# ziyaad30/ForwardTacotron

Hardware: AMD Instinct MI355X
Metric: mel_frames_per_sec_train_step (higher is better)
Workload: dtype f32

## Files before the change

### forwardtacotron_amd/csrc/ft_rnn_persist.hip

```cpp
#include <stdio.h>
#include <stdlib.h>
#include <string.h>

#include <mutex>
#include <vector>

#include "ft_rnn.h"

namespace {

constexpr int NSH = 16;
constexpr int CSTRIDE = 32;
constexpr unsigned MAX_SPINS_DEFAULT = 1u << 18;
constexpr int MB = 16;
constexpr int NFLAG = 256;
constexpr int NXCC = 64;

typedef unsigned int u32x4 __attribute__((ext_vector_type(4)));
typedef __bf16 bf16x8 __attribute__((ext_vector_type(8)));
typedef unsigned short u16x8 __attribute__((ext_vector_type(8)));

typedef __bf16 bf16x2v __attribute__((ext_vector_type(2)));
__device__ __forceinline__ unsigned rn_pack(float a, float b) {
  const bf16x2v p = {(__bf16)a, (__bf16)b};
  return __builtin_bit_cast(unsigned, p);
}
__device__ __forceinline__ void split_pair(float a, float b, unsigned& hi, unsigned& mid, unsigned& lo) {
  hi = rn_pack(a, b);
  const float a1 = a - __uint_as_float(hi << 16), b1 = b - __uint_as_float(hi & 0xFFFF0000u);
// ... 147 lines not shown
    same &= __hip_atomic_load(ids + i, __ATOMIC_RELAXED, __HIP_MEMORY_SCOPE_AGENT) == mine;
  return __all(same);
}

__device__ __forceinline__ bool decode(const Geom& g, int& d, int& bgp, int& chunk, int& grp) {
  const int lin = blockIdx.x, per = gridDim.x >> 3;
  const int w = g.xcd_aware ? (((lin & 7) + 8 - g.xcd_off) & 7) * per + (lin >> 3) : lin;
  if (w >= g.total) return false;
  grp = w / g.nchunks;
  chunk = w - grp * g.nchunks;
  d = grp / g.nbg;
  bgp = grp - d * g.nbg;
  return true;
}

template <int G, int NW, bool B3, int UB, int BC>
__global__ __launch_bounds__(NW * 64, NW == 4 ? 2 : 1) void ft_rnn_fwd_persist_kernel(RnnFwdArgs a, Geom geo, float* xb, unsigned* cnt,
                                                                     unsigned* fault, unsigned xb_bytes) {
  constexpr int NT = (G * UB + 15) / 16, BCH = BC, CW = UB / 4;
  constexpr bool GRAN = B3 && BC <= 2;
  static_assert(UB % 4 == 0 && CW <= NW, "cell waves");
  __shared__ float red2[2 * NW * NT * 16 * RLD];
  __shared__ int s_ok;
  int d, bgp, chunk, grp;
  if (!decode(geo, d, bgp, chunk, grp)) return;
  const int u0 = chunk * UB, b0 = bgp * MB;
  const int tid = threadIdx.x, wave = tid >> 6, lane = tid & 63;
  const int q = lane >> 4, l15 = lane & 15;
  const int H = a.H, T = a.T, nq = H / 4;
  const long ldo = (long)a.ND * H;
  const long ldx = (long)a.ND * G * H;
  const long grp_floats = (long)nq * MB * 4;
  const long par_floats = (long)2 * geo.nbg * grp_floats;
  const long base_floats = (long)grp * grp_floats;
  unsigned* mycnt = cnt + (long)grp * NSH * CSTRIDE;
  const int nprod = (geo.sig_per_wave ? CW : 1) * geo.nchunks;
  const __amdgpu_buffer_rsrc_t rs = __builtin_amdgcn_make_buffer_rsrc(xb, 0, (int)xb_bytes, 0x00020000);
  unsigned* myflags = cnt + (long)2 * geo.nbg * NSH * CSTRIDE + (long)grp * NFLAG;
  unsigned* myxcc = cnt + (long)2 * geo.nbg * (NSH * CSTRIDE + NFLAG) + (long)grp * NXCC;
  const unsigned my_xcc = xcc_id() + 1u;
  __shared__ int s_local, s_fail;
  bool local = false;
  if (tid == 0) {
// ... 26 lines not shown
        const bool in = valid && kb0 + c < kb1;
        const float* p = brow + (in ? 32 * (kb0 + c) + 8 * q : 0);
        const float4 z = make_float4(0, 0, 0, 0);
        split8(in ? *reinterpret_cast<const float4*>(p) : z, in ? *reinterpret_cast<const float4*>(p + 4) : z,
               bw[nt][c][0], bw[nt][c][1], bw[nt][c][2]);
      }
    }
  }

  const int pq0 = B3 ? 8 * kb0 : 4 * g0, pnq = B3 ? 8 * max(kb1 - kb0, 0) : 4 * max(g1 - g0, 0);
  const unsigned* pollf = lane < pnq ? myflags + pq0 + lane : nullptr;

  const int jq = tid >> 6, ci = (tid >> 2) & 15, jj = tid & 3;
  const int cu = 4 * jq + jj;
  const int cb = b0 + ci, cun = u0 + cu;
  const bool sthr = tid < 64 * CW;
  const bool cthr = sthr && cb < a.B;
  const int L = cthr ? clamp_len(a.lens, cb, T) : 0;
  float bg[G];
#pragma unroll
  for (int g = 0; g < G; ++g) bg[g] = sthr ? a.bhh[d][g * H + cun] : 0.f;
  float hprev = 0.f, cprev = 0.f;
  float xg[G];
#pragma unroll
  for (int g = 0; g < G; ++g) xg[g] = 0.f;
  const bool gated = a.gate != nullptr;
  int gate_off = 0;
  unsigned gate_have = 1u;
  if (gated && d == 1) {
    int lm = T;
    for (int i = 0; i < MB; ++i)
// ... 48 lines not shown
      for (int e = 0; e < 4; ++e) acc[nt][e] = 0.f;
    float4 av[B3 ? 1 : GCH];
    float4 aw[B3 ? BCH : 1][2];
    float xn[G];
#pragma unroll
    for (int g = 0; g < G; ++g) xn[g] = 0.f;
    auto request_xn = [&]() {
      if (cthr && s + 1 < L) xload(d == 0 ? s + 1 : L - 2 - s, xn);
    };
    const bool gl = local;
    const bool gm = GRAN && s > 0 && gl && geo.gran;
    const unsigned want_hi = ((unsigned)s & 0xFFFFu) << 16;
    const unsigned gbase = (unsigned)(((long)2 * par_floats * 4) + ((long)((s - 1) & 1) * par_floats + base_floats) * 8);
    auto goffs = [&](int c, unsigned& oa, unsigned& ob) {
      const long quad = 8 * (kb0 + c) + 2 * q;
      oa = gbase + (unsigned)((quad * MB + l15) * 4 * 8);
      ob = gbase + (unsigned)(((quad + 1) * MB + l15) * 4 * 8);
    };
    Gran gr[2];
    if (s > 0 && !gm) {
      if (gl) {
        if (!poll_flag(pollf, (unsigned)s, geo.max_spins) && lane == 0) s_fail = 1;
      } else {
        if (wave == 0) {
          const bool ok = wait_arrivals(mycnt, (unsigned)s, nprod, lane, geo.max_spins);
          if (s == 1 && ok && geo.local_ok) {
            const bool same = same_xcd(myxcc, geo.nchunks, my_xcc, lane);
            if (lane == 0) s_local = same;
          }
          if (lane == 0) s_ok = ok;
        }
        __syncthreads();
// ... 2 lines not shown
          return;
        }
        if (s == 1) {
          local = s_local != 0;
          if (threadIdx.x == 0 && chunk == 0) atomicAdd(fault + (local ? 8 : 9), 1u);
        }
      }
    }
    if (s > 0) {
      const long rbase = (long)((s - 1) & 1) * par_floats + base_floats;
      if constexpr (!B3) {
#pragma unroll
        for (int c = 0; c < GCH; ++c)
          if (g0 + c < g1) {
            const long quad = 4 * (g0 + c) + q;
            av[c] = ld_sc1_b128(rs, (unsigned)((rbase + (quad * MB + l15) * 4) * 4));
          }
        request_xn();
#pragma unroll
        for (int c = 0; c < GCH; ++c)
          if (g0 + c < g1) {
#pragma unroll
            for (int nt = 0; nt < NT; ++nt) mfma4(av[c], bv[nt][c], acc[nt]);
          }
      } else {
        if (gm) {
          if constexpr (GRAN) {
            if (kb0 < kb1) {
              unsigned oa, ob;
              goffs(0, oa, ob);
              gran_load(gr[0], rs, oa, ob);
            }
          }
        } else {
#pragma unroll
          for (int c = 0; c < BCH; ++c)
            if (kb0 + c < kb1) {
              const long quad = 8 * (kb0 + c) + 2 * q;
              aw[c][0] = ld_sc1_b128(rs, (unsigned)((rbase + (quad * MB + l15) * 4) * 4));
              aw[c][1] = ld_sc1_b128(rs, (unsigned)((rbase + ((quad + 1) * MB + l15) * 4) * 4));
            }
          request_xn();
        }
        bool ok = true;
#pragma unroll
        for (int c = 0; c < BCH; ++c)
          if (kb0 + c < kb1) {
            bf16x8 a3[3];
            if (gm) {
              if constexpr (GRAN) {
                unsigned oa, ob;
                if (c + 1 < BCH && kb0 + c + 1 < kb1) {
                  goffs(c + 1, oa, ob);
                  gran_load(gr[(c + 1) & 1], rs, oa, ob);
                }
// ... 57 lines not shown
      } else if (local) {
        __hip_atomic_store(xb + xe, hnew, __ATOMIC_RELAXED, __HIP_MEMORY_SCOPE_WAVEFRONT);
      } else {
        __hip_atomic_store(xb + xe, hnew, __ATOMIC_RELAXED, __HIP_MEMORY_SCOPE_AGENT);
      }
    }
    PROF(4);
    if (local && GRAN && geo.gran) {
      if (sthr) {
        const long xe = (long)(s & 1) * par_floats + base_floats + (((long)CW * chunk + jq) * MB + ci) * 4 + jj;
        unsigned long long* gp = reinterpret_cast<unsigned long long*>(xb + 2 * par_floats) + xe;
        __hip_atomic_store(gp, gran_make(cact ? hnew : 0.f, (unsigned)(s + 1) & 0xFFFFu), __ATOMIC_RELAXED,
                           __HIP_MEMORY_SCOPE_WAVEFRONT);
      }
    } else if (geo.sig_per_wave) {
      if (sthr) {
        asm volatile("s_waitcnt vmcnt(0)" ::: "memory");
        if (lane == 0) {
          if (local)
            __hip_atomic_store(myflags + CW * chunk + jq, (unsigned)(s + 1), __ATOMIC_RELAXED, __HIP_MEMORY_SCOPE_WAVEFRONT);
          else
            __hip_atomic_fetch_add(mycnt + ((CW * chunk + jq) % NSH) * CSTRIDE, 1u, __ATOMIC_RELAXED,
                                   __HIP_MEMORY_SCOPE_AGENT);
        }
      }
    } else {
      asm volatile("s_waitcnt vmcnt(0)" ::: "memory");
      __syncthreads();
      if (tid == 0)
        __hip_atomic_fetch_add(mycnt + (chunk % NSH) * CSTRIDE, 1u, __ATOMIC_RELAXED, __HIP_MEMORY_SCOPE_AGENT);
    }
// ... 13 lines not shown
    }
    PROF(6);
#pragma unroll
    for (int g = 0; g < G; ++g) xg[g] = xn[g];
    PROF(7);
  }
  PROF_DUMP(grp == 0 && chunk == 3 && wave == 0, 0);
  PROF_DUMP(grp == 0 && chunk == 3 && wave == NW - 1, 1);
}

template <int G, int NW, int GW, bool B3>
__global__ __launch_bounds__(NW * 64) void ft_rnn_bwd_persist_kernel(RnnBwdArgs a, Geom geo, float* xb, unsigned* cnt,
                                                                     unsigned* fault, unsigned xb_bytes) {
  __shared__ float red2[2 * NW * 16 * RLD];
  __shared__ int s_ok;
  int d, bgp, chunk, grp;
  if (!decode(geo, d, bgp, chunk, grp)) return;
  const int u0 = chunk * 16, b0 = bgp * MB;
  const int tid = threadIdx.x, wave = tid >> 6, lane = tid & 63;
  const int q = lane >> 4, l15 = lane & 15;
  const int H = a.H, T = a.T, K = G * H, nq = K / 4;
  const long ldg = (long)a.ND * K;
  const long ldo = (long)a.ND * H;
  const long grp_floats = (long)nq * MB * 4;
  const long par_floats = (long)2 * geo.nbg * grp_floats;
  const long base_floats = (long)grp * grp_floats;
  unsigned* mycnt = cnt + (long)grp * NSH * CSTRIDE;
  const int nprod = (geo.sig_per_wave ? 4 : 1) * geo.nchunks;
  const __amdgpu_buffer_rsrc_t rs = __builtin_amdgcn_make_buffer_rsrc(xb, 0, (int)xb_bytes, 0x00020000);
  unsigned* myflags = cnt + (long)2 * geo.nbg * NSH * CSTRIDE + (long)grp * NFLAG;
// ... 267 lines not shown
      if (G == 3) {
        float* dhh = a.dhp + ((long)s * a.B + cb) * ldg + (long)d * K + cun;
        dhh[0] = 0.f; dhh[H] = 0.f; dhh[2 * H] = 0.f;
      }
    }
    PROF(6);
#pragma unroll
    for (int g = 0; g < 4; ++g) gv[g] = ngv[g];
    dov = ndo; cc = ncc; prev = nprev;
    PROF(7);
  }
  PROF_DUMP(grp == 0 && chunk == 3 && wave == 0, 0);
  PROF_DUMP(grp == 0 && chunk == 3 && wave == 5, 1);
}

template <int G, int NW, int NT>
__global__ __launch_bounds__(NW * 64) void ft_rnn_bwd_rs_kernel(RnnBwdArgs a, Geom geo, float* xb, unsigned* cnt,
                                                                unsigned* fault, unsigned xb_bytes) {
  constexpr int ALD = 68;
  constexpr int GWV = 4;
  constexpr int TPW = NW * NT / GWV;
  constexpr bool PF = NW >= 8;
  constexpr int NIN = 7;
  __shared__ __attribute__((aligned(16))) float adg2[2 * 16 * ALD];
  __shared__ __attribute__((aligned(16))) float rsum[GWV * 256];
  __shared__ float inb[PF ? 2 * NIN * 256 : 1];
  __shared__ int s_ok;
  int d, bgp, chunk, grp;
  if (!decode(geo, d, bgp, chunk, grp)) return;
  const int u0 = chunk * 16, b0 = bgp * MB;
  const int tid = threadIdx.x, wave = tid >> 6, lane = tid & 63;
  const int q = lane >> 4, l15 = lane & 15;
  const int H = a.H, T = a.T, K = G * H, P = geo.nchunks;
  const long ldg = (long)a.ND * K;
  const long ldo = (long)a.ND * H;
  const long grp_floats = (long)P * P * 256;
  const long par_floats = (long)2 * geo.nbg * grp_floats;
  const long base_floats = (long)grp * grp_floats;
  unsigned* mycnt = cnt + (long)grp * NSH * CSTRIDE;
  const int nprod = NW * P;
  const __amdgpu_buffer_rsrc_t rs = __builtin_amdgcn_make_buffer_rsrc(xb, 0, (int)xb_bytes, 0x00020000);
  unsigned* myflags = cnt + (long)2 * geo.nbg * NSH * CSTRIDE + (long)grp * NFLAG;
  unsigned* myxcc = cnt + (long)2 * geo.nbg * (NSH * CSTRIDE + NFLAG) + (long)grp * NXCC;
  const unsigned my_xcc = xcc_id() + 1u;
  __shared__ int s_local, s_fail;
  bool local = false;
  if (threadIdx.x == 0) {
    s_local = 0;
    s_fail = 0;
    __hip_atomic_store(myxcc + chunk, my_xcc, __ATOMIC_RELAXED, __HIP_MEMORY_SCOPE_AGENT);
  }

  bf16x8 bw[NT][2][3];
#pragma unroll
  for (int nt = 0; nt < NT; ++nt) {
    const int n = (wave * NT + nt) * 16 + l15;
#pragma unroll
    for (int blk = 0; blk < 2; ++blk) {
      const int g = 2 * blk + (q >> 1), j0 = 8 * (q & 1);
      const bool in = g < G && n < H;
      const float* p = a.whhT[d] + (in ? (long)n * K + (long)g * H + u0 + j0 : 0);
      const float4 z = make_float4(0, 0, 0, 0);
      split8(in ? *reinterpret_cast<const float4*>(p) : z, in ? *reinterpret_cast<const float4*>(p + 4) : z,
             bw[nt][blk][0], bw[nt][blk][1], bw[nt][blk][2]);
    }
  }
  for (int i = tid; i < 2 * 16 * ALD; i += NW * 64) adg2[i] = 0.f;

  const unsigned* pollf =
      (wave < GWV && lane < TPW && wave * TPW + lane < P) ? myflags + NW * (wave * TPW + lane) + chunk / NT : nullptr;

  const int cj = tid >> 4, ci = tid & 15;
  const int cb = b0 + ci, cun = u0 + cj;
  const bool sthr = tid < 256;
  const bool cthr = sthr && cb < a.B;
  const int L = cthr ? clamp_len(a.lens, cb, T) : 0;
  float carry = 0.f;
  const bool fwave = PF && wave == 4;
  const int fr = lane >> 2, fq = lane & 3;
  const int fb = b0 + fr;
  const int FL = (fwave && fb < a.B) ? clamp_len(a.lens, fb, T) : 0;

  float gv[4] = {0.f, 0.f, 0.f, 0.f}, dov = 0.f, cc = 0.f, prev = 0.f;
  auto request = [&](int sn, float (&rgv)[4], float& rdo, float& rcc, float& rprev) {
#pragma unroll
    for (int g = 0; g < 4; ++g) rgv[g] = 0.f;
    rdo = 0.f; rcc = 0.f; rprev = 0.f;
    if (cthr && sn < L) {
      const int ct = d == 0 ? L - 1 - sn : sn;
      const int tprev = d == 0 ? ct - 1 : ct + 1;
      const bool has_prev = tprev >= 0 && tprev < L;
      const long o = ((long)ct * a.B + cb) * ldo + (long)d * H + cun;
      const long op = ((long)tprev * a.B + cb) * ldo + (long)d * H + cun;
      const float* gs = a.gates + (((long)ct * a.B + cb) * a.ND + d) * 4 * H + cun;
#pragma unroll
      for (int g = 0; g < 4; ++g) rgv[g] = gs[(long)g * H];
      rdo = a.dout[o];
      if (G == 3) {
        rprev = has_prev ? a.out[op] : 0.f;
      } else {
        rcc = a.cst[o];
        rprev = has_prev ? a.cst[op] : 0.f;
      }
    }
  };
  float4 fv[NIN];
#pragma unroll
  for (int i = 0; i < NIN; ++i) fv[i] = make_float4(0.f, 0.f, 0.f, 0.f);
  auto fetch = [&](int sn) {
#pragma unroll
    for (int i = 0; i < NIN; ++i) fv[i] = make_float4(0.f, 0.f, 0.f, 0.f);
    if (fwave && sn < FL) {
      const int ct = d == 0 ? FL - 1 - sn : sn;
      const int tprev = d == 0 ? ct - 1 : ct + 1;
      const bool has_prev = tprev >= 0 && tprev < FL;
      const long o = ((long)ct * a.B + fb) * ldo + (long)d * H + u0 + 4 * fq;
      const long op = ((long)tprev * a.B + fb) * ldo + (long)d * H + u0 + 4 * fq;
      const float* gs = a.gates + (((long)ct * a.B + fb) * a.ND + d) * 4 * H + u0 + 4 * fq;
#pragma unroll
      for (int g = 0; g < 4; ++g) fv[g] = *reinterpret_cast<const float4*>(gs + (long)g * H);
      fv[4] = *reinterpret_cast<const float4*>(a.dout + o);
      if (G == 3) {
        if (has_prev) fv[6] = *reinterpret_cast<const float4*>(a.out + op);
      } else {
        fv[5] = *reinterpret_cast<const float4*>(a.cst + o);
        if (has_prev) fv[6] = *reinterpret_cast<const float4*>(a.cst + op);
      }
    }
  };
  auto publish = [&](int sn) {
    if (fwave) {
      float* ib = inb + (sn & 1) * (NIN * 256) + (4 * fq) * 16 + fr;
#pragma unroll
      for (int i = 0; i < NIN; ++i) {
        ib[i * 256] = fv[i].x; ib[i * 256 + 16] = fv[i].y; ib[i * 256 + 32] = fv[i].z; ib[i * 256 + 48] = fv[i].w;
      }
    }
  };
  if constexpr (PF) {
    fetch(0);
    publish(0);
  } else {
    request(0, gv, dov, cc, prev);
  }
  __syncthreads();
  PROF_DECL;

  for (int s = 0; s < T; ++s) {
    PROF(0);
    const bool cact = cthr && s < L;
    const int ct = d == 0 ? L - 1 - s : s;
    float* adg = adg2 + (s & 1) * (16 * ALD);
    float rec = 0.f;
    if (s > 0) {
      if (local) {
        if (!poll_flag(pollf, (unsigned)s, geo.max_spins) && lane == 0) s_fail = 1;
      } else {
        if (wave == 0) {
          const bool ok = wait_arrivals(mycnt, (unsigned)s, nprod, lane, geo.max_spins);
          if (s == 1 && ok && geo.local_ok) {
            const bool same = same_xcd(myxcc, P, my_xcc, lane);
            if (lane == 0) s_local = same;
          }
          if (lane == 0) s_ok = ok;
        }
        __syncthreads();
        if (!s_ok) {
          if (tid == 0) atomicExch(fault, 1u);
          return;
        }
        if (s == 1) {
          local = s_local != 0;
          if (threadIdx.x == 0 && chunk == 0) atomicAdd(fault + (local ? 8 : 9), 1u);
        }
      }
      PROF(1);
      if (wave < GWV) {
        const long rbase = (long)((s - 1) & 1) * par_floats + base_floats + (long)chunk * P * 256 + 4 * lane;
        float4 v[TPW];
#pragma unroll
        for (int i = 0; i < TPW; ++i) {
          const int pp = wave * TPW + i;
          v[i] = pp < P ? ld_sc1_b128(rs, (unsigned)((rbase + (long)pp * 256) * 4)) : make_float4(0.f, 0.f, 0.f, 0.f);
        }
        float4 acc4 = v[0];
#pragma unroll
        for (int i = 1; i < TPW; ++i) {
          acc4.x += v[i].x; acc4.y += v[i].y; acc4.z += v[i].z; acc4.w += v[i].w;
        }
        *reinterpret_cast<float4*>(rsum + wave * 256 + 4 * lane) = acc4;
      }
      __syncthreads();
      if (sthr) {
#pragma unroll
        for (int w = 0; w < GWV; ++w) rec += rsum[w * 256 + tid];
      }
    }
    if constexpr (PF) {
      fetch(s + 1);
      if (sthr) {
        const float* ib = inb + (s & 1) * (NIN * 256) + tid;
#pragma unroll
        for (int g = 0; g < 4; ++g) gv[g] = ib[g * 256];
        dov = ib[4 * 256]; cc = ib[5 * 256]; prev = ib[6 * 256];
      }
    }
    float ngv[4] = {0.f, 0.f, 0.f, 0.f}, ndo = 0.f, ncc = 0.f, nprev = 0.f;
    if constexpr (!PF) request(s + 1, ngv, ndo, ncc, nprev);
#ifdef FT_RNN_PROF
    asm volatile("" : "+v"(rec));
#endif
    PROF(2);

    float dgx[4] = {0.f, 0.f, 0.f, 0.f}, dgh2 = 0.f;
    if (cact) {
      if (G == 3) {
        const float dh = dov + rec + carry;
        const float r = gv[0], z = gv[1], n = gv[2], hn = gv[3];
        const float dz = dh * (prev - n) * z * (1.f - z);
// ... 19 lines not shown
#pragma unroll
      for (int g = 0; g < G; ++g) adg[ci * ALD + g * 16 + cj] = (G == 3 && g == 2) ? dgh2 : dgx[g];
    }
    PROF(3);
    __syncthreads();
    PROF(4);
    if (s_fail) {
      if (tid == 0) atomicExch(fault, 1u);
      return;
    }

    if (s + 1 < T) {
      bf16x8 a3[2][3];
#pragma unroll
      for (int blk = 0; blk < 2; ++blk) {
        const float* ap = adg + l15 * ALD + 32 * blk + 8 * q;
        split8(*reinterpret_cast<const float4*>(ap), *reinterpret_cast<const float4*>(ap + 4), a3[blk][0], a3[blk][1],
               a3[blk][2]);
      }
      PROF(5);
      const long wbase = (long)(s & 1) * par_floats + base_floats + (long)chunk * 256 + l15 * 16 + 4 * q;
#pragma unroll
      for (int nt = 0; nt < NT; ++nt) {
        f32x4 acc = {0.f, 0.f, 0.f, 0.f};
        mfma6(a3[0], bw[nt][0], acc);
        mfma6(a3[1], bw[nt][1], acc);
        const int cons = wave * NT + nt;
        if (cons < P) {
          u32x4 v = {__float_as_uint(acc[0]), __float_as_uint(acc[1]), __float_as_uint(acc[2]), __float_as_uint(acc[3])};
          const unsigned off = (unsigned)((wbase + (long)cons * P * 256) * 4);
          if (local) __builtin_amdgcn_raw_buffer_store_b128(v, rs, off, 0, 0);
          else __builtin_amdgcn_raw_buffer_store_b128(v, rs, off, 0, 16);
        }
      }
      PROF(6);
      asm volatile("s_waitcnt vmcnt(0)" ::: "memory");
      PROF(7);
      if (lane == 0) {
        if (local)
          __hip_atomic_store(myflags + NW * chunk + wave, (unsigned)(s + 1), __ATOMIC_RELAXED, __HIP_MEMORY_SCOPE_WAVEFRONT);
        else
          __hip_atomic_fetch_add(mycnt + ((NW * chunk + wave) % NSH) * CSTRIDE, 1u, __ATOMIC_RELAXED,
                                 __HIP_MEMORY_SCOPE_AGENT);
      }
    }
// ... 46 lines not shown
  if (!cus) {
    int dev = 0;
    hipDeviceProp_t p;
    if (hipGetDevice(&dev) == hipSuccess && hipGetDeviceProperties(&p, dev) == hipSuccess) cus = p.multiProcessorCount;
    if (cus <= 0) cus = 1;
  }
  return cus;
}

struct PersistWs {
  float* xb;
  unsigned* cnt;
  size_t sync_bytes, xb_bytes, total_bytes;
};
size_t sync_region_bytes(int ngrp) { return (size_t)ngrp * (NSH * CSTRIDE + NFLAG + NXCC) * sizeof(unsigned); }
PersistWs carve_ws(void* ws, int ngrp, int K) {
  PersistWs p;
  p.sync_bytes = sync_region_bytes(ngrp);
  p.cnt = (unsigned*)ws;
  p.xb_bytes = (size_t)3 * 2 * ngrp * (K / 4) * MB * 4 * sizeof(float);
  p.xb = (float*)((char*)ws + p.sync_bytes);
  p.total_bytes = p.sync_bytes + p.xb_bytes;
  return p;
}

PersistWs carve_ws_rs(void* ws, int ngrp, int nchunks) {
  PersistWs p;
  p.sync_bytes = sync_region_bytes(ngrp);
  p.cnt = (unsigned*)ws;
  p.xb_bytes = (size_t)2 * ngrp * nchunks * nchunks * 256 * sizeof(float);
  p.xb = (float*)((char*)ws + p.sync_bytes);
  p.total_bytes = p.sync_bytes + p.xb_bytes;
  return p;
}

constexpr int MAX_DEV = 16;
unsigned g_max_spins = MAX_SPINS_DEFAULT;
long g_n_persistent = 0, g_n_refused = 0, g_n_waited = 0;

int current_device() {
  int dev = 0;
  if (hipGetDevice(&dev) != hipSuccess || dev < 0 || dev >= MAX_DEV) dev = 0;
  return dev;
}

struct Flight {
  hipEvent_t ev;
  hipStream_t stream;
// ... 108 lines not shown
              geo.total, geo.nchunks, cand[i].aligned ? "aligned" : "spread", cand[i].per, d, ok ? "admitted" : "refused");
    if (!ok) continue;
    grid = cand[i].grid;
    geo.xcd_off = cand[i].xcd_off;
    geo.local_ok = cand[i].aligned && env_int("FT_RNN_LOCAL", 1);
    geo.gran = env_int("FT_RNN_GRANULES", 1);
    geo.fast = env_int("FT_RNN_FAST_CELL", 1);
    return d;
  }
  ++g_n_refused;
  return -1.0;
}

double* g_fill_probe = nullptr;

template <int G, int NW, bool B3, int UB, int BC>
int launch_fwd_persist(const RnnFwdArgs& a, Geom geo, const PersistWs& p, hipStream_t stream) {
  if (g_fill_probe) {
    const int ngroups = geo.total / geo.nchunks;
    *g_fill_probe = xcd_demand(ft_rnn_fwd_persist_kernel<G, NW, B3, UB, BC>, NW * 64, geo.nchunks * ft_cdiv(ngroups, 8));
    return FT_OK;
  }
  int grid = 0;
  const double cus = plan_launch(ft_rnn_fwd_persist_kernel<G, NW, B3, UB, BC>, NW * 64, geo, grid, stream);
  if (cus < 0.0) return -1;
  if (BC > 2 && !env_int("FT_RNN_GRAN4", 1)) geo.gran = 0;
  (void)hipMemsetAsync(p.cnt, 0, p.total_bytes, stream);
  hipLaunchKernelGGL((ft_rnn_fwd_persist_kernel<G, NW, B3, UB, BC>), dim3(grid), dim3(NW * 64), 0, stream, a, geo, p.xb,
                     p.cnt, ft_rnn_fault_word(), (unsigned)p.xb_bytes);
  admitted_launch_done(cus, stream);
  return ft_check_launch("rnn_fwd_persistent");
}

template <int G>
int fwd_persistent(RnnFwdArgs a, void* ws, size_t ws_bytes, hipStream_t stream) {
  if (!persistent_enabled() || !ws || a.T < 2) return -1;
  const int H = a.H, B = a.B;
  if (!a.vec || H % 16 != 0) return -1;
  const int ngroups = H / 16;
  int NW = ngroups > 16 ? 8 : 4;
  const bool wide = NW == 8 && G == 4 && H / 8 > 32 && H % 32 == 0 && ft_cdiv(H / 32, 8) <= 2 && env_int("FT_RNN_B3", 1) &&
                    env_int("FT_RNN_FWD_UB16", 1);
  if (!wide && NW == 8 && G == 4 && H % 32 == 0 && ft_cdiv(H / 32, 4) <= 4 && env_int("FT_RNN_FWD_NW4", 1)) NW = 4;
  if (ft_cdiv(ngroups, NW) > GCH) return -1;
  const int bpw = H % 32 == 0 ? ft_cdiv(H / 32, NW) : 99;
  const bool b3 = bpw <= 4 && env_int("FT_RNN_B3", 1);
  const bool gru_wide = G == 3 && H == 256 && b3 && NW == 4 && env_int("FT_RNN_GRU_WIDE", 1);
  Geom geo;
  geo.nchunks = H / ((wide || gru_wide) ? 16 : 8);
  geo.nbg = ft_cdiv(B, MB);
  geo.total = a.ND * geo.nbg * geo.nchunks;
  geo.xcd_aware = env_int("FT_RNN_XCDMAP", 1);
  geo.sig_per_wave = env_int("FT_RNN_SIG", 1);
  geo.max_spins = g_max_spins;
  PersistWs p = carve_ws(ws, 2 * geo.nbg, H);
  if (ws_bytes < p.total_bytes || p.xb_bytes >= (1ull << 31)) return -1;
  geo.xcd_off = 0;
  geo.local_ok = 0;
  geo.gran = 0;
  geo.fast = 0;
  a.s = 0;
  if (wide) return launch_fwd_persist<G, 8, true, 16, 2>(a, geo, p, stream);
  if constexpr (G == 3) {
    if (gru_wide) return launch_fwd_persist<G, 8, true, 16, 1>(a, geo, p, stream);
  }
  if (b3) {
    if (NW == 8) return bpw <= 1 ? launch_fwd_persist<G, 8, true, 8, 1>(a, geo, p, stream)
                                 : launch_fwd_persist<G, 8, true, 8, 2>(a, geo, p, stream);
    if (bpw <= 1) return launch_fwd_persist<G, 4, true, 8, 1>(a, geo, p, stream);
    if (bpw <= 2) return launch_fwd_persist<G, 4, true, 8, 2>(a, geo, p, stream);
    return launch_fwd_persist<G, 4, true, 8, 4>(a, geo, p, stream);
  }
  return NW == 8 ? launch_fwd_persist<G, 8, false, 8, 1>(a, geo, p, stream)
                 : launch_fwd_persist<G, 4, false, 8, 1>(a, geo, p, stream);
}

// ... 2 lines not shown
  if (g_fill_probe) {
    *g_fill_probe = xcd_demand(ft_rnn_bwd_persist_kernel<G, NW, GW, B3>, NW * 64,
                               geo.nchunks * ft_cdiv(geo.total / geo.nchunks, 8));
    return FT_OK;
  }
  int grid = 0;
  const double cus = plan_launch(ft_rnn_bwd_persist_kernel<G, NW, GW, B3>, NW * 64, geo, grid, stream);
  if (cus < 0.0) return -1;
  (void)hipMemsetAsync(p.cnt, 0, p.total_bytes, stream);
  hipLaunchKernelGGL((ft_rnn_bwd_persist_kernel<G, NW, GW, B3>), dim3(grid), dim3(NW * 64), 0, stream, a, geo, p.xb, p.cnt,
                     ft_rnn_fault_word(), (unsigned)p.xb_bytes);
  admitted_launch_done(cus, stream);
  return ft_check_launch("rnn_bwd_persistent");
}

template <int G, int NW, int NT>
int launch_bwd_rs(const RnnBwdArgs& a, Geom geo, const PersistWs& p, hipStream_t stream) {
  if (g_fill_probe) {
    *g_fill_probe = xcd_demand(ft_rnn_bwd_rs_kernel<G, NW, NT>, NW * 64, geo.nchunks * ft_cdiv(geo.total / geo.nchunks, 8));
    return FT_OK;
  }
  int grid = 0;
  const double cus = plan_launch(ft_rnn_bwd_rs_kernel<G, NW, NT>, NW * 64, geo, grid, stream);
  if (cus < 0.0) return -1;
  (void)hipMemsetAsync(p.cnt, 0, p.sync_bytes, stream);
  hipLaunchKernelGGL((ft_rnn_bwd_rs_kernel<G, NW, NT>), dim3(grid), dim3(NW * 64), 0, stream, a, geo, p.xb, p.cnt,
                     ft_rnn_fault_word(), (unsigned)p.xb_bytes);
  admitted_launch_done(cus, stream);
  return ft_check_launch("rnn_bwd_persistent_rs");
}

template <int G>
int bwd_persistent_rs(RnnBwdArgs a, const Geom& geo, void* ws, size_t ws_bytes, hipStream_t stream) {
  const int tiles = a.H / 16;
  if (!env_int("FT_RNN_BWD_RS", 1) || !env_int("FT_RNN_B3", 1) || !geo.sig_per_wave) return -1;
  PersistWs p = carve_ws_rs(ws, 2 * geo.nbg, geo.nchunks);
  if (ws_bytes < p.total_bytes || p.xb_bytes >= (1ull << 31)) return -1;
  const bool force = env_int("FT_RNN_BWD_RS", 1) == 2;
  if (!force && G * a.H < 1024) return -1;
  switch (tiles) {
    case 4: return launch_bwd_rs<G, 4, 1>(a, geo, p, stream);
    case 8: return launch_bwd_rs<G, 8, 1>(a, geo, p, stream);
    case 16: return launch_bwd_rs<G, 8, 2>(a, geo, p, stream);
    case 32: return launch_bwd_rs<G, 8, 4>(a, geo, p, stream);
    default: return -1;
  }
}

template <int G>
int bwd_persistent(RnnBwdArgs a, void* ws, size_t ws_bytes, hipStream_t stream) {
  if (!persistent_enabled() || !ws || a.T < 2) return -1;
  const int H = a.H, B = a.B, K = G * H;
  if (!a.vec || H % 16 != 0) return -1;
  const int ngroups = K / 16;
  const int NW = ngroups > 128 ? 16 : (ngroups > 16 ? 8 : 4);
  const int GW = ngroups > 64 ? 16 : 8;
  if (ft_cdiv(ngroups, NW) > GW) return -1;
  Geom geo;
  geo.nchunks = H / 16;
  geo.nbg = ft_cdiv(B, MB);
  geo.total = 2 * geo.nbg * geo.nchunks;
  geo.xcd_aware = env_int("FT_RNN_XCDMAP", 1);
  geo.sig_per_wave = env_int("FT_RNN_SIG", 1);
  geo.max_spins = g_max_spins;
  geo.xcd_off = 0;
  geo.local_ok = 0;
  geo.gran = 0;
  geo.fast = 0;
  a.s = 0;
  {
    const int rc = bwd_persistent_rs<G>(a, geo, ws, ws_bytes, stream);
    if (rc != -1) return rc;
  }
  PersistWs p = carve_ws(ws, 2 * geo.nbg, K);
  if (ws_bytes < p.total_bytes || p.xb_bytes >= (1ull << 31)) return -1;
  if (K % 32 == 0 && ft_cdiv(K / 32, NW) <= GW / 2 && env_int("FT_RNN_B3", 1)) {
    if (NW == 16) return launch_bwd_persist<G, 16, 16, true>(a, geo, p, stream);
    if (NW == 8) return GW == 16 ? launch_bwd_persist<G, 8, 16, true>(a, geo, p, stream)
                                 : launch_bwd_persist<G, 8, 8, true>(a, geo, p, stream);
    return launch_bwd_persist<G, 4, 8, true>(a, geo, p, stream);
  }
  if (NW == 16) return launch_bwd_persist<G, 16, 16, false>(a, geo, p, stream);
  if (NW == 8) return GW == 16 ? launch_bwd_persist<G, 8, 16, false>(a, geo, p, stream)
                               : launch_bwd_persist<G, 8, 8, false>(a, geo, p, stream);
  return launch_bwd_persist<G, 4, 8, false>(a, geo, p, stream);
}

}

// ... 33 lines not shown
  g_fill_probe = nullptr;
  return rc == FT_OK ? fill : -1.0;
}

int ft_rnn_fwd_persistent(int G, RnnFwdArgs a, void* ws, size_t ws_bytes, hipStream_t stream) {
  return G == 3 ? fwd_persistent<3>(a, ws, ws_bytes, stream) : fwd_persistent<4>(a, ws, ws_bytes, stream);
}
int ft_rnn_bwd_persistent(int G, RnnBwdArgs a, void* ws, size_t ws_bytes, hipStream_t stream) {
  return G == 3 ? bwd_persistent<3>(a, ws, ws_bytes, stream) : bwd_persistent<4>(a, ws, ws_bytes, stream);
}

extern "C" {

size_t ft_rnn_workspace(int gates, int B, int H) {
  if (gates < 3 || gates > 4 || B <= 0 || H <= 0 || H % 16 != 0) return 0;
  const int ngrp = 2 * ft_cdiv(B, MB);
  const PersistWs f = carve_ws(nullptr, ngrp, H);
  const PersistWs b = carve_ws(nullptr, ngrp, gates * H);
  const PersistWs r = carve_ws_rs(nullptr, ngrp, H / 16);
  size_t m = f.total_bytes > b.total_bytes ? f.total_bytes : b.total_bytes;
  return r.total_bytes > m ? r.total_bytes : m;
}

int ft_rnn_xcd_fill_pct(int gates, int backward, int B, int T, int H) {
  if ((gates != 3 && gates != 4) || B <= 0 || H <= 0) return -1;
  void* const ws = (void*)(uintptr_t)256;
  const double f = backward ? ft_rnn_bwd_xcd_fill(gates, B, T, H, ws, (size_t)-1)
                            : ft_rnn_fwd_xcd_fill(gates, B, T, H, ws, (size_t)-1);
  return f < 0.0 ? -1 : (int)(f * 100.0 + 0.5);
}
int ft_rnn_admit_budget_pct(void) { return (int)(0.75 * env_int("FT_RNN_ADMIT_PCT", 100) + 0.5); }

int ft_rnn_set_persistent(int enabled) {
  int old = persistent_enabled() ? 1 : 0;
  g_persistent = enabled ? 1 : 0;
  return old;
// ... 65 lines not shown
```

Before: 951,000.

## Add 8-row-per-workgroup variant for wide LSTM persistent RNN kernels

Templates the forward persistent kernel and the backward reduce-scatter kernel on the batch rows per workgroup (MB), and adds an 8-row variant for 4-gate LSTMs with H=512. A heuristic picks 8 rows when small batches would otherwise fill fewer than 8 groups, so more workgroups share the recurrence and the per-step work per group shrinks. Workspace sizing and shared buffers scale with MB. In exchange there are more groups to synchronise, MFMA lanes go partly idle, and per-group efficiency is lower.

```diff
diff --git a/forwardtacotron_amd/csrc/ft_rnn_persist.hip b/forwardtacotron_amd/csrc/ft_rnn_persist.hip
--- a/forwardtacotron_amd/csrc/ft_rnn_persist.hip
+++ b/forwardtacotron_amd/csrc/ft_rnn_persist.hip
@@ -12,7 +12,7 @@
 constexpr int NSH = 16;
 constexpr int CSTRIDE = 32;
 constexpr unsigned MAX_SPINS_DEFAULT = 1u << 18;
-constexpr int MB = 16;
+constexpr int MB16 = 16;
 constexpr int NFLAG = 256;
 constexpr int NXCC = 64;
 
@@ -190,12 +190,13 @@
   return true;
 }
 
-template <int G, int NW, bool B3, int UB, int BC>
+template <int G, int NW, bool B3, int UB, int BC, int MB>
 __global__ __launch_bounds__(NW * 64, NW == 4 ? 2 : 1) void ft_rnn_fwd_persist_kernel(RnnFwdArgs a, Geom geo, float* xb, unsigned* cnt,
                                                                      unsigned* fault, unsigned xb_bytes) {
   constexpr int NT = (G * UB + 15) / 16, BCH = BC, CW = UB / 4;
   constexpr bool GRAN = B3 && BC <= 2;
   static_assert(UB % 4 == 0 && CW <= NW, "cell waves");
+  static_assert(MB == 16 || MB == 8, "rows per workgroup");
   __shared__ float red2[2 * NW * NT * 16 * RLD];
   __shared__ int s_ok;
   int d, bgp, chunk, grp;
@@ -203,6 +204,7 @@
   const int u0 = chunk * UB, b0 = bgp * MB;
   const int tid = threadIdx.x, wave = tid >> 6, lane = tid & 63;
   const int q = lane >> 4, l15 = lane & 15;
+  const int ar = l15 & (MB - 1);
   const int H = a.H, T = a.T, nq = H / 4;
   const long ldo = (long)a.ND * H;
   const long ldx = (long)a.ND * G * H;
@@ -259,7 +261,8 @@
   const int jq = tid >> 6, ci = (tid >> 2) & 15, jj = tid & 3;
   const int cu = 4 * jq + jj;
   const int cb = b0 + ci, cun = u0 + cu;
-  const bool sthr = tid < 64 * CW;
+  const bool cwave = tid < 64 * CW;
+  const bool sthr = cwave && ci < MB;
   const bool cthr = sthr && cb < a.B;
   const int L = cthr ? clamp_len(a.lens, cb, T) : 0;
   float bg[G];
@@ -338,8 +341,8 @@
     const unsigned gbase = (unsigned)(((long)2 * par_floats * 4) + ((long)((s - 1) & 1) * par_floats + base_floats) * 8);
     auto goffs = [&](int c, unsigned& oa, unsigned& ob) {
       const long quad = 8 * (kb0 + c) + 2 * q;
-      oa = gbase + (unsigned)((quad * MB + l15) * 4 * 8);
-      ob = gbase + (unsigned)(((quad + 1) * MB + l15) * 4 * 8);
+      oa = gbase + (unsigned)((quad * MB + ar) * 4 * 8);
+      ob = gbase + (unsigned)(((quad + 1) * MB + ar) * 4 * 8);
     };
     Gran gr[2];
     if (s > 0 && !gm) {
@@ -372,7 +375,7 @@
         for (int c = 0; c < GCH; ++c)
           if (g0 + c < g1) {
             const long quad = 4 * (g0 + c) + q;
-            av[c] = ld_sc1_b128(rs, (unsigned)((rbase + (quad * MB + l15) * 4) * 4));
+            av[c] = ld_sc1_b128(rs, (unsigned)((rbase + (quad * MB + ar) * 4) * 4));
           }
         request_xn();
 #pragma unroll
@@ -395,8 +398,8 @@
           for (int c = 0; c < BCH; ++c)
             if (kb0 + c < kb1) {
               const long quad = 8 * (kb0 + c) + 2 * q;
-              aw[c][0] = ld_sc1_b128(rs, (unsigned)((rbase + (quad * MB + l15) * 4) * 4));
-              aw[c][1] = ld_sc1_b128(rs, (unsigned)((rbase + ((quad + 1) * MB + l15) * 4) * 4));
+              aw[c][0] = ld_sc1_b128(rs, (unsigned)((rbase + (quad * MB + ar) * 4) * 4));
+              aw[c][1] = ld_sc1_b128(rs, (unsigned)((rbase + ((quad + 1) * MB + ar) * 4) * 4));
             }
           request_xn();
         }
@@ -484,7 +487,7 @@
                            __HIP_MEMORY_SCOPE_WAVEFRONT);
       }
     } else if (geo.sig_per_wave) {
-      if (sthr) {
+      if (cwave) {
         asm volatile("s_waitcnt vmcnt(0)" ::: "memory");
         if (lane == 0) {
           if (local)
@@ -528,6 +531,7 @@
                                                                      unsigned* fault, unsigned xb_bytes) {
   __shared__ float red2[2 * NW * 16 * RLD];
   __shared__ int s_ok;
+  constexpr int MB = MB16;
   int d, bgp, chunk, grp;
   if (!decode(geo, d, bgp, chunk, grp)) return;
   const int u0 = chunk * 16, b0 = bgp * MB;
@@ -825,7 +829,7 @@
   PROF_DUMP(grp == 0 && chunk == 3 && wave == 5, 1);
 }
 
-template <int G, int NW, int NT>
+template <int G, int NW, int NT, int MB>
 __global__ __launch_bounds__(NW * 64) void ft_rnn_bwd_rs_kernel(RnnBwdArgs a, Geom geo, float* xb, unsigned* cnt,
                                                                 unsigned* fault, unsigned xb_bytes) {
   constexpr int ALD = 68;
@@ -833,9 +837,11 @@
   constexpr int TPW = NW * NT / GWV;
   constexpr bool PF = NW >= 8;
   constexpr int NIN = 7;
-  __shared__ __attribute__((aligned(16))) float adg2[2 * 16 * ALD];
-  __shared__ __attribute__((aligned(16))) float rsum[GWV * 256];
-  __shared__ float inb[PF ? 2 * NIN * 256 : 1];
+  static_assert(MB == 16 || MB == 8, "rows per workgroup");
+  constexpr int TS = 16 * MB;
+  __shared__ __attribute__((aligned(16))) float adg2[2 * MB * ALD];
+  __shared__ __attribute__((aligned(16))) float rsum[GWV * TS];
+  __shared__ float inb[PF ? 2 * NIN * TS : 1];
   __shared__ int s_ok;
   int d, bgp, chunk, grp;
   if (!decode(geo, d, bgp, chunk, grp)) return;
@@ -845,7 +851,7 @@
   const int H = a.H, T = a.T, K = G * H, P = geo.nchunks;
   const long ldg = (long)a.ND * K;
   const long ldo = (long)a.ND * H;
-  const long grp_floats = (long)P * P * 256;
+  const long grp_floats = (long)P * P * TS;
   const long par_floats = (long)2 * geo.nbg * grp_floats;
   const long base_floats = (long)grp * grp_floats;
   unsigned* mycnt = cnt + (long)grp * NSH * CSTRIDE;
@@ -876,21 +882,22 @@
              bw[nt][blk][0], bw[nt][blk][1], bw[nt][blk][2]);
     }
   }
-  for (int i = tid; i < 2 * 16 * ALD; i += NW * 64) adg2[i] = 0.f;
+  for (int i = tid; i < 2 * MB * ALD; i += NW * 64) adg2[i] = 0.f;
 
   const unsigned* pollf =
       (wave < GWV && lane < TPW && wave * TPW + lane < P) ? myflags + NW * (wave * TPW + lane) + chunk / NT : nullptr;
 
-  const int cj = tid >> 4, ci = tid & 15;
+  const int cj = tid / MB, ci = tid % MB;
   const int cb = b0 + ci, cun = u0 + cj;
-  const bool sthr = tid < 256;
+  const bool sthr = tid < TS;
   const bool cthr = sthr && cb < a.B;
   const int L = cthr ? clamp_len(a.lens, cb, T) : 0;
   float carry = 0.f;
   const bool fwave = PF && wave == 4;
   const int fr = lane >> 2, fq = lane & 3;
+  const bool flane = fwave && fr < MB;
   const int fb = b0 + fr;
-  const int FL = (fwave && fb < a.B) ? clamp_len(a.lens, fb, T) : 0;
+  const int FL = (flane && fb < a.B) ? clamp_len(a.lens, fb, T) : 0;
 
   float gv[4] = {0.f, 0.f, 0.f, 0.f}, dov = 0.f, cc = 0.f, prev = 0.f;
   auto request = [&](int sn, float (&rgv)[4], float& rdo, float& rcc, float& rprev) {
@@ -921,7 +928,7 @@
   auto fetch = [&](int sn) {
 #pragma unroll
     for (int i = 0; i < NIN; ++i) fv[i] = make_float4(0.f, 0.f, 0.f, 0.f);
-    if (fwave && sn < FL) {
+    if (flane && sn < FL) {
       const int ct = d == 0 ? FL - 1 - sn : sn;
       const int tprev = d == 0 ? ct - 1 : ct + 1;
       const bool has_prev = tprev >= 0 && tprev < FL;
@@ -940,11 +947,11 @@
     }
   };
   auto publish = [&](int sn) {
-    if (fwave) {
-      float* ib = inb + (sn & 1) * (NIN * 256) + (4 * fq) * 16 + fr;
+    if (flane) {
+      float* ib = inb + (sn & 1) * (NIN * TS) + (4 * fq) * MB + fr;
 #pragma unroll
       for (int i = 0; i < NIN; ++i) {
-        ib[i * 256] = fv[i].x; ib[i * 256 + 16] = fv[i].y; ib[i * 256 + 32] = fv[i].z; ib[i * 256 + 48] = fv[i].w;
+        ib[i * TS] = fv[i].x; ib[i * TS + MB] = fv[i].y; ib[i * TS + 2 * MB] = fv[i].z; ib[i * TS + 3 * MB] = fv[i].w;
       }
     }
   };
@@ -961,7 +968,7 @@
     PROF(0);
     const bool cact = cthr && s < L;
     const int ct = d == 0 ? L - 1 - s : s;
-    float* adg = adg2 + (s & 1) * (16 * ALD);
+    float* adg = adg2 + (s & 1) * (MB * ALD);
     float rec = 0.f;
     if (s > 0) {
       if (local) {
@@ -986,34 +993,34 @@
         }
       }
       PROF(1);
-      if (wave < GWV) {
-        const long rbase = (long)((s - 1) & 1) * par_floats + base_floats + (long)chunk * P * 256 + 4 * lane;
+      if (wave < GWV && 4 * lane < TS) {
+        const long rbase = (long)((s - 1) & 1) * par_floats + base_floats + (long)chunk * P * TS + 4 * lane;
         float4 v[TPW];
 #pragma unroll
         for (int i = 0; i < TPW; ++i) {
           const int pp = wave * TPW + i;
-          v[i] = pp < P ? ld_sc1_b128(rs, (unsigned)((rbase + (long)pp * 256) * 4)) : make_float4(0.f, 0.f, 0.f, 0.f);
+          v[i] = pp < P ? ld_sc1_b128(rs, (unsigned)((rbase + (long)pp * TS) * 4)) : make_float4(0.f, 0.f, 0.f, 0.f);
         }
         float4 acc4 = v[0];
 #pragma unroll
         for (int i = 1; i < TPW; ++i) {
           acc4.x += v[i].x; acc4.y += v[i].y; acc4.z += v[i].z; acc4.w += v[i].w;
         }
-        *reinterpret_cast<float4*>(rsum + wave * 256 + 4 * lane) = acc4;
+        *reinterpret_cast<float4*>(rsum + wave * TS + 4 * lane) = acc4;
       }
       __syncthreads();
       if (sthr) {
 #pragma unroll
-        for (int w = 0; w < GWV; ++w) rec += rsum[w * 256 + tid];
+        for (int w = 0; w < GWV; ++w) rec += rsum[w * TS + tid];
       }
     }
     if constexpr (PF) {
       fetch(s + 1);
       if (sthr) {
-        const float* ib = inb + (s & 1) * (NIN * 256) + tid;
-#pragma unroll
-        for (int g = 0; g < 4; ++g) gv[g] = ib[g * 256];
-        dov = ib[4 * 256]; cc = ib[5 * 256]; prev = ib[6 * 256];
+        const float* ib = inb + (s & 1) * (NIN * TS) + tid;
+#pragma unroll
+        for (int g = 0; g < 4; ++g) gv[g] = ib[g * TS];
+        dov = ib[4 * TS]; cc = ib[5 * TS]; prev = ib[6 * TS];
       }
     }
     float ngv[4] = {0.f, 0.f, 0.f, 0.f}, ndo = 0.f, ncc = 0.f, nprev = 0.f;
@@ -1063,21 +1070,21 @@
       bf16x8 a3[2][3];
 #pragma unroll
       for (int blk = 0; blk < 2; ++blk) {
-        const float* ap = adg + l15 * ALD + 32 * blk + 8 * q;
+        const float* ap = adg + (l15 & (MB - 1)) * ALD + 32 * blk + 8 * q;
         split8(*reinterpret_cast<const float4*>(ap), *reinterpret_cast<const float4*>(ap + 4), a3[blk][0], a3[blk][1],
                a3[blk][2]);
       }
       PROF(5);
-      const long wbase = (long)(s & 1) * par_floats + base_floats + (long)chunk * 256 + l15 * 16 + 4 * q;
+      const long wbase = (long)(s & 1) * par_floats + base_floats + (long)chunk * TS + l15 * MB + 4 * q;
 #pragma unroll
       for (int nt = 0; nt < NT; ++nt) {
         f32x4 acc = {0.f, 0.f, 0.f, 0.f};
         mfma6(a3[0], bw[nt][0], acc);
         mfma6(a3[1], bw[nt][1], acc);
         const int cons = wave * NT + nt;
-        if (cons < P) {
+        if (cons < P && 4 * q < MB) {
           u32x4 v = {__float_as_uint(acc[0]), __float_as_uint(acc[1]), __float_as_uint(acc[2]), __float_as_uint(acc[3])};
-          const unsigned off = (unsigned)((wbase + (long)cons * P * 256) * 4);
+          const unsigned off = (unsigned)((wbase + (long)cons * P * TS) * 4);
           if (local) __builtin_amdgcn_raw_buffer_store_b128(v, rs, off, 0, 0);
           else __builtin_amdgcn_raw_buffer_store_b128(v, rs, off, 0, 16);
         }
@@ -1154,24 +1161,30 @@
   size_t sync_bytes, xb_bytes, total_bytes;
 };
 size_t sync_region_bytes(int ngrp) { return (size_t)ngrp * (NSH * CSTRIDE + NFLAG + NXCC) * sizeof(unsigned); }
-PersistWs carve_ws(void* ws, int ngrp, int K) {
+PersistWs carve_ws(void* ws, int ngrp, int K, int mb) {
   PersistWs p;
   p.sync_bytes = sync_region_bytes(ngrp);
   p.cnt = (unsigned*)ws;
-  p.xb_bytes = (size_t)3 * 2 * ngrp * (K / 4) * MB * 4 * sizeof(float);
+  p.xb_bytes = (size_t)3 * 2 * ngrp * (K / 4) * mb * 4 * sizeof(float);
   p.xb = (float*)((char*)ws + p.sync_bytes);
   p.total_bytes = p.sync_bytes + p.xb_bytes;
   return p;
 }
 
-PersistWs carve_ws_rs(void* ws, int ngrp, int nchunks) {
+PersistWs carve_ws_rs(void* ws, int ngrp, int nchunks, int mb) {
   PersistWs p;
   p.sync_bytes = sync_region_bytes(ngrp);
   p.cnt = (unsigned*)ws;
-  p.xb_bytes = (size_t)2 * ngrp * nchunks * nchunks * 256 * sizeof(float);
+  p.xb_bytes = (size_t)2 * ngrp * nchunks * nchunks * 16 * mb * sizeof(float);
   p.xb = (float*)((char*)ws + p.sync_bytes);
   p.total_bytes = p.sync_bytes + p.xb_bytes;
   return p;
+}
+
+int rows_per_wg(int nd, int B) {
+  if (env_int("FT_RNN_MB", 8) == 16) return 16;
+  const int g16 = nd * ft_cdiv(B, 16), g8 = nd * ft_cdiv(B, 8);
+  return g16 < 8 && g8 <= 8 && g8 > g16 ? 8 : 16;
 }
 
 constexpr int MAX_DEV = 16;
@@ -1310,19 +1323,19 @@
 
 double* g_fill_probe = nullptr;
 
-template <int G, int NW, bool B3, int UB, int BC>
+template <int G, int NW, bool B3, int UB, int BC, int MB = MB16>
 int launch_fwd_persist(const RnnFwdArgs& a, Geom geo, const PersistWs& p, hipStream_t stream) {
   if (g_fill_probe) {
     const int ngroups = geo.total / geo.nchunks;
-    *g_fill_probe = xcd_demand(ft_rnn_fwd_persist_kernel<G, NW, B3, UB, BC>, NW * 64, geo.nchunks * ft_cdiv(ngroups, 8));
+    *g_fill_probe = xcd_demand(ft_rnn_fwd_persist_kernel<G, NW, B3, UB, BC, MB>, NW * 64, geo.nchunks * ft_cdiv(ngroups, 8));
     return FT_OK;
   }
   int grid = 0;
-  const double cus = plan_launch(ft_rnn_fwd_persist_kernel<G, NW, B3, UB, BC>, NW * 64, geo, grid, stream);
+  const double cus = plan_launch(ft_rnn_fwd_persist_kernel<G, NW, B3, UB, BC, MB>, NW * 64, geo, grid, stream);
   if (cus < 0.0) return -1;
   if (BC > 2 && !env_int("FT_RNN_GRAN4", 1)) geo.gran = 0;
   (void)hipMemsetAsync(p.cnt, 0, p.total_bytes, stream);
-  hipLaunchKernelGGL((ft_rnn_fwd_persist_kernel<G, NW, B3, UB, BC>), dim3(grid), dim3(NW * 64), 0, stream, a, geo, p.xb,
+  hipLaunchKernelGGL((ft_rnn_fwd_persist_kernel<G, NW, B3, UB, BC, MB>), dim3(grid), dim3(NW * 64), 0, stream, a, geo, p.xb,
                      p.cnt, ft_rnn_fault_word(), (unsigned)p.xb_bytes);
   admitted_launch_done(cus, stream);
   return ft_check_launch("rnn_fwd_persistent");
@@ -1342,20 +1355,24 @@
   const int bpw = H % 32 == 0 ? ft_cdiv(H / 32, NW) : 99;
   const bool b3 = bpw <= 4 && env_int("FT_RNN_B3", 1);
   const bool gru_wide = G == 3 && H == 256 && b3 && NW == 4 && env_int("FT_RNN_GRU_WIDE", 1);
+  const int mb = wide && G == 4 ? rows_per_wg(a.ND, B) : MB16;
   Geom geo;
   geo.nchunks = H / ((wide || gru_wide) ? 16 : 8);
-  geo.nbg = ft_cdiv(B, MB);
+  geo.nbg = ft_cdiv(B, mb);
   geo.total = a.ND * geo.nbg * geo.nchunks;
   geo.xcd_aware = env_int("FT_RNN_XCDMAP", 1);
   geo.sig_per_wave = env_int("FT_RNN_SIG", 1);
   geo.max_spins = g_max_spins;
-  PersistWs p = carve_ws(ws, 2 * geo.nbg, H);
+  PersistWs p = carve_ws(ws, 2 * geo.nbg, H, mb);
   if (ws_bytes < p.total_bytes || p.xb_bytes >= (1ull << 31)) return -1;
   geo.xcd_off = 0;
   geo.local_ok = 0;
   geo.gran = 0;
   geo.fast = 0;
   a.s = 0;
+  if constexpr (G == 4) {
+    if (wide && mb == 8) return launch_fwd_persist<G, 8, true, 16, 2, 8>(a, geo, p, stream);
+  }
   if (wide) return launch_fwd_persist<G, 8, true, 16, 2>(a, geo, p, stream);
   if constexpr (G == 3) {
     if (gru_wide) return launch_fwd_persist<G, 8, true, 16, 1>(a, geo, p, stream);
@@ -1388,27 +1405,31 @@
   return ft_check_launch("rnn_bwd_persistent");
 }
 
-template <int G, int NW, int NT>
+template <int G, int NW, int NT, int MB = MB16>
 int launch_bwd_rs(const RnnBwdArgs& a, Geom geo, const PersistWs& p, hipStream_t stream) {
   if (g_fill_probe) {
-    *g_fill_probe = xcd_demand(ft_rnn_bwd_rs_kernel<G, NW, NT>, NW * 64, geo.nchunks * ft_cdiv(geo.total / geo.nchunks, 8));
+    *g_fill_probe =
+        xcd_demand(ft_rnn_bwd_rs_kernel<G, NW, NT, MB>, NW * 64, geo.nchunks * ft_cdiv(geo.total / geo.nchunks, 8));
     return FT_OK;
   }
   int grid = 0;
-  const double cus = plan_launch(ft_rnn_bwd_rs_kernel<G, NW, NT>, NW * 64, geo, grid, stream);
+  const double cus = plan_launch(ft_rnn_bwd_rs_kernel<G, NW, NT, MB>, NW * 64, geo, grid, stream);
   if (cus < 0.0) return -1;
   (void)hipMemsetAsync(p.cnt, 0, p.sync_bytes, stream);
-  hipLaunchKernelGGL((ft_rnn_bwd_rs_kernel<G, NW, NT>), dim3(grid), dim3(NW * 64), 0, stream, a, geo, p.xb, p.cnt,
+  hipLaunchKernelGGL((ft_rnn_bwd_rs_kernel<G, NW, NT, MB>), dim3(grid), dim3(NW * 64), 0, stream, a, geo, p.xb, p.cnt,
                      ft_rnn_fault_word(), (unsigned)p.xb_bytes);
   admitted_launch_done(cus, stream);
   return ft_check_launch("rnn_bwd_persistent_rs");
 }
 
 template <int G>
-int bwd_persistent_rs(RnnBwdArgs a, const Geom& geo, void* ws, size_t ws_bytes, hipStream_t stream) {
+int bwd_persistent_rs(RnnBwdArgs a, Geom geo, void* ws, size_t ws_bytes, hipStream_t stream) {
   const int tiles = a.H / 16;
   if (!env_int("FT_RNN_BWD_RS", 1) || !env_int("FT_RNN_B3", 1) || !geo.sig_per_wave) return -1;
-  PersistWs p = carve_ws_rs(ws, 2 * geo.nbg, geo.nchunks);
+  const int mb = G == 4 && tiles == 32 ? rows_per_wg(2, a.B) : MB16;
+  geo.nbg = ft_cdiv(a.B, mb);
+  geo.total = 2 * geo.nbg * geo.nchunks;
+  PersistWs p = carve_ws_rs(ws, 2 * geo.nbg, geo.nchunks, mb);
   if (ws_bytes < p.total_bytes || p.xb_bytes >= (1ull << 31)) return -1;
   const bool force = env_int("FT_RNN_BWD_RS", 1) == 2;
   if (!force && G * a.H < 1024) return -1;
@@ -1416,7 +1437,11 @@
     case 4: return launch_bwd_rs<G, 4, 1>(a, geo, p, stream);
     case 8: return launch_bwd_rs<G, 8, 1>(a, geo, p, stream);
     case 16: return launch_bwd_rs<G, 8, 2>(a, geo, p, stream);
-    case 32: return launch_bwd_rs<G, 8, 4>(a, geo, p, stream);
+    case 32:
+      if constexpr (G == 4) {
+        if (mb == 8) return launch_bwd_rs<G, 8, 4, 8>(a, geo, p, stream);
+      }
+      return launch_bwd_rs<G, 8, 4>(a, geo, p, stream);
     default: return -1;
   }
 }
@@ -1432,7 +1457,7 @@
   if (ft_cdiv(ngroups, NW) > GW) return -1;
   Geom geo;
   geo.nchunks = H / 16;
-  geo.nbg = ft_cdiv(B, MB);
+  geo.nbg = ft_cdiv(B, MB16);
   geo.total = 2 * geo.nbg * geo.nchunks;
   geo.xcd_aware = env_int("FT_RNN_XCDMAP", 1);
   geo.sig_per_wave = env_int("FT_RNN_SIG", 1);
@@ -1446,7 +1471,7 @@
     const int rc = bwd_persistent_rs<G>(a, geo, ws, ws_bytes, stream);
     if (rc != -1) return rc;
   }
-  PersistWs p = carve_ws(ws, 2 * geo.nbg, K);
+  PersistWs p = carve_ws(ws, 2 * geo.nbg, K, MB16);
   if (ws_bytes < p.total_bytes || p.xb_bytes >= (1ull << 31)) return -1;
   if (K % 32 == 0 && ft_cdiv(K / 32, NW) <= GW / 2 && env_int("FT_RNN_B3", 1)) {
     if (NW == 16) return launch_bwd_persist<G, 16, 16, true>(a, geo, p, stream);
@@ -1510,12 +1535,17 @@
 
 size_t ft_rnn_workspace(int gates, int B, int H) {
   if (gates < 3 || gates > 4 || B <= 0 || H <= 0 || H % 16 != 0) return 0;
-  const int ngrp = 2 * ft_cdiv(B, MB);
-  const PersistWs f = carve_ws(nullptr, ngrp, H);
-  const PersistWs b = carve_ws(nullptr, ngrp, gates * H);
-  const PersistWs r = carve_ws_rs(nullptr, ngrp, H / 16);
-  size_t m = f.total_bytes > b.total_bytes ? f.total_bytes : b.total_bytes;
-  return r.total_bytes > m ? r.total_bytes : m;
+  size_t m = 0;
+  for (int mb : {MB16, 8}) {
+    const int ngrp = 2 * ft_cdiv(B, mb);
+    const size_t f = carve_ws(nullptr, ngrp, H, mb).total_bytes;
+    const size_t b = carve_ws(nullptr, ngrp, gates * H, mb).total_bytes;
+    const size_t r = carve_ws_rs(nullptr, ngrp, H / 16, mb).total_bytes;
+    m = f > m ? f : m;
+    m = b > m ? b : m;
+    m = r > m ? r : m;
+  }
+  return m;
 }
 
 int ft_rnn_xcd_fill_pct(int gates, int backward, int B, int T, int H) {
diff --git a/lab/rnn_rows_us.py b/lab/rnn_rows_us.py
--- /dev/null
+++ b/lab/rnn_rows_us.py
@@ -0,0 +1,47 @@
+import os, statistics, sys, torch
+sys.path.insert(0, '.')
+from forwardtacotron_amd import hip as H
+dev = 'cuda'
+B = int(sys.argv[1]) if len(sys.argv) > 1 else 32
+T = int(sys.argv[2]) if len(sys.argv) > 2 else 841
+reps = int(sys.argv[3]) if len(sys.argv) > 3 else 7
+Hh = 512
+g = torch.Generator().manual_seed(0)
+xp = (torch.randn(T, B, 8 * Hh, generator=g) * 0.1).to(dev)
+whh = [(torch.randn(4 * Hh, Hh, generator=g) * 0.03).to(dev) for _ in range(2)]
+bhh = [torch.zeros(4 * Hh, device=dev) for _ in range(2)]
+dout = (torch.randn(T, B, 2 * Hh, generator=g) * 0.1).to(dev)
+lens = torch.randint(T // 2, T + 1, (B,), generator=g)
+lens[0] = T
+lens = lens.to(dev)
+wt = [H.transpose2d(w) for w in whh]
+
+
+def timed(f):
+    s, e = torch.cuda.Event(enable_timing=True), torch.cuda.Event(enable_timing=True)
+    s.record(); r = f(); e.record(); torch.cuda.synchronize()
+    return s.elapsed_time(e) * 1e3 / T, r
+
+
+us = {mb: ([], []) for mb in (16, 8)}
+res = {}
+for rep in range(reps + 1):
+    for mb in (16, 8):
+        os.environ['FT_RNN_MB'] = str(mb)
+        m0 = H.rnn_mode_counts()
+        tf, (raw, cst, gates) = timed(lambda: H.lstm_fwd(xp, whh[0], whh[1], bhh[0], bhh[1], lens, Hh, True))
+        tb, dg = timed(lambda: H.lstm_bwd(dout, raw, cst, gates, wt[0], wt[1], lens, Hh))
+        m1 = H.rnn_mode_counts()
+        if rep == 0:
+            res[mb] = ((raw, cst, gates, dg), (m1[0] - m0[0], m1[1] - m0[1]))
+            continue
+        us[mb][0].append(tf)
+        us[mb][1].append(tb)
+H.check_rnn_status()
+same = [torch.equal(a, b) for a, b in zip(res[8][0], res[16][0])]
+for mb in (16, 8):
+    f, b = us[mb]
+    print(f'LSTM-512 B{B} T{T} MB={mb:2d}: fwd {statistics.median(f):.3f} us/step (min {min(f):.3f} max {max(f):.3f}) | '
+          f'bwd {statistics.median(b):.3f} (min {min(b):.3f} max {max(b):.3f}) | groups local/agent {res[mb][1]}', flush=True)
+print('bit-equal out/cst/gates/dg:', same)
+print('persistent/refused', H.rnn_counters())
```

Result: faster. 1.000 million, median of 6 (+5.2%).
